# subtotechnoblade/Grok_Alpha_Zero

Measured on AMD Instinct MI355X. Metric: self-play positions/sec (whole node), Connect4 200 sims/move, 1/2/4/8 GPU, higher is better.
Workload: dtype bf16; 1 GPU; Connect4 6x7, 4096 concurrent games/GPU, 200 sims/move (MCTS.run iteration_limit), 6-block x128 ResNet bf16, puct self-play, random-init weights; games_per_gpu=4096, sims_per_move=200, evaluator=resnet

## Files before the change

grok_alpha_zero_amd/build.py:

```python
import os
import subprocess
from concurrent.futures import ThreadPoolExecutor

_PKG = os.path.dirname(os.path.abspath(__file__))
CSRC = os.path.join(_PKG, "csrc")
OBJ = os.path.join(CSRC, "build")
LIB = os.path.join(_PKG, "libgaz_engine.so")
HEADER = os.path.join(os.path.dirname(_PKG), "include", "gaz_engine.h")
UNITS = {
    "engine.hip": ["rt.hpp", "wave.hpp", "det.hpp", "games.hpp", "tree.hpp", "puct_core.hpp", "gumbel_core.hpp", "evaluator.hpp", "samples.hpp", "tree_export.hpp"],
    "resnet.hip": ["rt.hpp", "wave.hpp", "evaluator.hpp", "netops.hpp", "conv3x3.hpp", "conv_wide.hpp", "resblock.hpp", "trunk.hpp", "tile_perm.hpp", "net_host.hpp",
                   "det.hpp", "games.hpp", "tree.hpp", "puct_core.hpp", "gumbel_core.hpp"],
}
FLAGS = ["-O3", "--offload-arch=gfx950", "-fPIC", "-std=c++17", "-ffp-contract=off", "-Wno-unused-result", "-Wno-unused-value",
         "-Wno-int-to-pointer-cast"]


def _newer(target, deps):
    if not os.path.exists(target):
        return True
    t = os.path.getmtime(target)
    return any(os.path.getmtime(d) > t for d in deps)


def build_engine(force=False, verbose=False):
    hipcc = os.environ.get("HIPCC", "/opt/rocm/bin/hipcc")
    os.makedirs(OBJ, exist_ok=True)
    known = {h for hs in UNITS.values() for h in hs} | set(UNITS)
    extra = [f for f in os.listdir(CSRC) if f.endswith((".hpp", ".hip")) and f not in known]
    jobs = []
    for src, hdrs in UNITS.items():
        obj = os.path.join(OBJ, src.replace(".hip", ".o"))
        deps = [os.path.join(CSRC, src), HEADER, os.path.abspath(__file__)] + [os.path.join(CSRC, h) for h in hdrs + extra]
        if force or _newer(obj, deps):
            jobs.append([hipcc] + FLAGS + ["-c", os.path.join(CSRC, src), "-o", obj])

    def run(cmd):
        if verbose:
            print(" ".join(cmd), flush=True)
        subprocess.check_call(cmd, cwd=CSRC)
    with ThreadPoolExecutor(max_workers=max(len(jobs), 1)) as ex:
        list(ex.map(run, jobs))
    objs = [os.path.join(OBJ, s.replace(".hip", ".o")) for s in UNITS]
    if jobs or _newer(LIB, objs):
        run([hipcc, "--offload-arch=gfx950", "-shared", "-fPIC"] + objs + ["-o", LIB])
# ... 2 lines not shown
```

grok_alpha_zero_amd/csrc/engine.hip:

```cpp
#include <stdio.h>
#include <functional>
#include <string>
#include <vector>
#include "../../include/gaz_engine.h"
#include "rt.hpp"
#include "puct_core.hpp"
#include "gumbel_core.hpp"
#include "samples.hpp"
#include "tree_export.hpp"
#include "evaluator.hpp"

using namespace gaz;

static std::string g_create_error;

#define HIP_OK(expr)                                                                  \
    do { hipError_t _e = (expr); if (_e != hipSuccess) { return fail(std::string(#expr) + ": " + hipGetErrorString(_e)); } } while (0)

template <class G> GAZ_DEV void wave_body(const DevParams<G>& E, int g0, int g1) {
    constexpr int PER = WAVE / G::TEAM;
    GAZ_SHARED Scratch<G> S[PER];
    GAZ_SHARED PuctLocal<G> L[PER];
    const int t = team_in_wave<G>();
    const int g = g0 + block_id() * PER + t;
    if (g < g1) game_step<G>(E, g, S[t], L[t]);
}
template <class G> GAZ_KERNEL k_wave(DevParams<G> E, int g0, int g1) { wave_body<G>(E, g0, g1); }
template <class G> GAZ_KERNEL_TEAMS k_wave_teams(DevParams<G> E, int g0, int g1) { wave_body<G>(E, g0, g1); }

template <class G> GAZ_DEV void wave_body_lb(const DevParams<G>& E, const LeafBatch& B, int g0, int g1) {
    constexpr int PER = WAVE / G::TEAM;
    GAZ_SHARED Scratch<G> S[PER];
    GAZ_SHARED PuctLocal<G> L[PER];
    const int t = team_in_wave<G>();
    const int g = g0 + block_id() * PER + t;
    if (g < g1) game_step_lb<G>(E, B, g, S[t], L[t]);
}
template <class G> GAZ_KERNEL_TEAMS k_wave_lb(DevParams<G> E, LeafBatch B, int g0, int g1) { wave_body_lb<G>(E, B, g0, g1); }

template <class G> GAZ_KERNEL k_gather_pending_lb(DevParams<G> E, int K, int32_t* out) {
    const int g = block_id();
    if (g >= E.n_games) return;
    const GameState<G>& gs = E.games[g];
    const int n = gs.pend_kind == PEND_ROOT ? 1 : (gs.pend_kind == PEND_EXPAND ? gs.pend_depth : 0);
    for (int j = lane_id(); j < K; j += WAVE) out[(size_t)g * K + j] = j < n ? gs.pend_kind : PEND_NONE;
}

template <class G> GAZ_KERNEL k_count_reserved(DevParams<G> E, unsigned long long* out) {
    const int g = block_id();
    if (g >= E.n_games) return;
    unsigned long long sum = 0;
    for (int t = 0; t < 2; ++t) {
        const int n = (int)E.trees[(size_t)g * 2 + t].n_nodes;
        for (int i = lane_id(); i < n; i += WAVE) sum += node_at(E, g, t, i).hdr()->pad[0];
    }
    if (sum) atomic_add(out, sum);
}

template <class G> GAZ_DEV void wave_body_gumbel(const DevParams<G>& E, int g0, int g1) {
    constexpr int PER = WAVE / G::TEAM;
    GAZ_SHARED Scratch<G> S[PER];
    GAZ_SHARED GumbelLocal<G> L[PER];
    const int t = team_in_wave<G>();
    const int g = g0 + block_id() * PER + t;
    if (g < g1) g_game_step<G>(E, g, S[t], L[t]);
}
template <class G> GAZ_KERNEL k_wave_gumbel(DevParams<G> E, int g0, int g1) { wave_body_gumbel<G>(E, g0, g1); }
template <class G> GAZ_KERNEL_TEAMS k_wave_gumbel_teams(DevParams<G> E, int g0, int g1) { wave_body_gumbel<G>(E, g0, g1); }

template <class G> GAZ_DEV void wave_body_gb(const DevParams<G>& E, const GumbelBatch& B, int g0, int g1) {
    constexpr int PER = WAVE / G::TEAM;
    GAZ_SHARED Scratch<G> S[PER];
    GAZ_SHARED GumbelLocal<G> L[PER];
    const int t = team_in_wave<G>();
    const int g = g0 + block_id() * PER + t;
    if (g < g1) g_game_step_gb<G>(E, B, g, S[t], L[t]);
}
template <class G> GAZ_KERNEL_TEAMS k_wave_gb(DevParams<G> E, GumbelBatch B, int g0, int g1) { wave_body_gb<G>(E, B, g0, g1); }

template <class G> GAZ_KERNEL k_gather_pending_gb(DevParams<G> E, GumbelBatch B, int32_t* out) {
    const int g = block_id();
    if (g >= E.n_games) return;
    const int kind = E.games[g].pend_kind;
    for (int j = lane_id(); j < B.K; j += WAVE)
        out[(size_t)g * B.K + j] = kind == PEND_ROOT ? (j == 0 ? PEND_ROOT : PEND_NONE) : (kind == PEND_EXPAND && B.rows[(size_t)g * B.K + j].pend ? PEND_EXPAND : PEND_NONE);
}

template <class G> GAZ_KERNEL k_cache_insert(DevParams<G> E, int g0, int g1) {
    const int g = g0 + block_id();
    if (g < g1) cache_insert<G>(E, g);
}

template <int UNUSED> GAZ_KERNEL_WIDE k_init_puct_table(double* table, double c_init, double c_base, int n) {
#ifdef GAZ_HOST_EMU
    for (int i = 0; i < n; ++i) { table[2 * i] = dsqrt((double)i); table[2 * i + 1] = puct_c_of((double)i, c_init, c_base); }
#else
    const int i = blockIdx.x * blockDim.x + threadIdx.x;
    if (i < n) { table[2 * i] = dsqrt((double)i); table[2 * i + 1] = puct_c_of((double)i, c_init, c_base); }
#endif
}

template <class G> GAZ_KERNEL k_init_games(DevParams<G> E, int first_seq) {
    const int g = block_id();
    if (g >= E.n_games || lane_id() != 0) return;
    GameState<G>& gs = E.games[g];
    memset(&gs, 0, sizeof(gs));
    gs.phase = (E.games_budget > 0 && (long long)g >= E.games_budget) ? PH_HALT : PH_NEW_GAME;
    gs.pend_kind = PEND_NONE; gs.game_seq = (uint32_t)first_seq; gs.host_move = -1; gs.winner = RUNNING;
    gs.slot_id = E.slot_offset + (uint32_t)g;
    E.trees[g * 2].root = -1; E.trees[g * 2 + 1].root = -1;
}

template <class G> GAZ_KERNEL k_reset_games(DevParams<G> E, const int32_t* slots, int n) {
    const int i = block_id();
    if (i >= n || lane_id() != 0) return;
    const int g = slots ? slots[i] : i;
    if (g < 0 || g >= E.n_games) return;
    GameState<G>& gs = E.games[g];
// ... 343 lines not shown
        if (dalloc(&E.paths, rows * PathCap<G>::V)) return 1;
        if (lbk > 1 && gbk <= 1) { LB.K = lbk; if (dalloc(&LB.pend, rows)) return 1; }
        if (gbk > 1) { GB.K = gbk; if (dalloc(&GB.rows, rows)) return 1; }
        if (gumbel) { GumbelState<G>* gp = nullptr; if (dalloc(&gp, (size_t)n)) return 1; E.gstate = gp; }
        if (dalloc(&E.recs, (size_t)n * RL::SIZE)) return 1;
        if (dalloc(&E.ring, (size_t)(cfg.ring_capacity > 0 ? cfg.ring_capacity : 1) * RL::SIZE)) return 1;
        if (dalloc(&E.ring_head, 4)) return 1;
        if (dalloc(&E.nn_in, rows * G::HW * G::C + 64)) return 1;
        if (dalloc(&E.nn_policy, rows * G::A + 64)) return 1;
        if (dalloc(&E.nn_value, rows + 64)) return 1;
        if (cfg.eval_cache_log2 < 0 || cfg.eval_cache_log2 > 28) return fail("eval_cache_log2 out of range (0 = off, at most 28)");
        if (cfg.eval_cache_log2 > 0) {
            const size_t slots = (size_t)1 << cfg.eval_cache_log2;
            E.cache_stride = CacheLayout<G>::SIZE; E.cache_mask = (uint32_t)(slots - 1); E.cache_epoch = 1;
            if (dalloc(&E.cache, slots * (size_t)E.cache_stride)) return 1;
            if (dalloc(&E.cache_lock, slots)) return 1;
        }
        if (getenv("GAZ_TREE_PROF") && atoi(getenv("GAZ_TREE_PROF"))) { if (dalloc(&E.prof, (size_t)n * 8)) return 1; }
        if (!gumbel) {
            double* tb = nullptr;
            if (dalloc(&tb, (size_t)2 * PUCT_TABLE_N)) return 1;
            E.puct_table = tb;
            if (init_puct_table()) return 1;
        }
        if (dalloc(&E.stats, 8)) return 1;
        if (dalloc(&E.error, 4)) return 1;
        if (dalloc(&dN, (size_t)n * G::A) || dalloc(&dW, (size_t)n * G::A) || dalloc(&dP, (size_t)n * G::A) ||
            dalloc(&dPol, (size_t)n * G::A) || dalloc(&dRV, n) || dalloc(&dQ, n) || dalloc(&dChosen, n) ||
            dalloc(&dPhase, n) || dalloc(&dPending, rows) || dalloc(&dCount, 16) || dalloc(&dMoves, (size_t)n + G::MAXT) || dalloc(&dSlots, n)) return 1;
        std::string e2;
        gaz_engine_config ecfg = cfg; ecfg.n_games = (int32_t)rows;
        eval = make_evaluator(ecfg, G::H, G::W, G::C, G::A, &e2);
        if (!eval && cfg.evaluator != GAZ_EVAL_EXTERNAL) return fail("evaluator: " + e2);
        GAZ_LAUNCH(k_init_games<G>, n, WAVE, stream, E, (int)cfg.first_game_seq);
        HIP_OK(hipGetLastError());
        HIP_OK(hipStreamSynchronize(stream));
        return 0;
    }

    void note_grouped() override { if (eval) eval->set_shared_chip(this->grouped > 1); }

    int check_device_error() {
        int32_t code = 0;
        HIP_OK(hipMemcpy(&code, E.error, sizeof(code), hipMemcpyDeviceToHost));
        if (code) {
            const char* names[] = {"", "tree arena full (raise nodes_per_tree)", "root not fully expanded at move end",
                                   "selection path longer than the game can last", "state-machine loop guard", "PUCT picked an un-poppable child"};
            return fail(std::string("device error: ") + (code > 0 && code < 6 ? names[code] : "unknown"));
        }
        return 0;
    }

    int load_weights(const gaz_tensor* t, int n) override {
        if (!eval) return fail("no evaluator to load weights into");
        std::string m;
        if (eval->load(t, n, stream, &m)) return fail("load_weights: " + m);
        if (E.cache) {
            HIP_OK(hipMemsetAsync(E.cache, 0, ((size_t)E.cache_mask + 1) * (size_t)E.cache_stride, stream));
            HIP_OK(hipStreamSynchronize(stream));
        }
        return 0;
    }

    int reset_games(const int32_t* slots, int n) override {
        if (slots && n_eff != E.n_games) return fail("reset_games(slots): not after gaz_engine_repack (a physical slot no longer identifies a game; reset all games instead)");
        if (!slots) n_eff = E.n_games;
// ... 113 lines not shown
        int n_active = 0;
        for (int g = 0; g < n_eff; ++g) n_active += ph[g] != PH_HALT;
        for (int g = n_eff; g < E.n_games; ++g) if (ph[g] != PH_HALT) return fail("repack: a slot beyond the live range is running");
        if (n_active_out) *n_active_out = n_active;
        const int n_new = n_active > 0 ? n_active : 1;
        std::vector<int32_t> mv;
        int hole = 0;
        for (int g = n_eff - 1; g >= n_new; --g) {
            if (ph[g] == PH_HALT) continue;
            while (hole < n_new && ph[hole] != PH_HALT) ++hole;
            if (hole >= n_new) return fail("repack: internal error (no hole left)");
            mv.push_back(g); mv.push_back(hole); ph[hole] = ph[g]; ph[g] = PH_HALT;
        }
        if (!mv.empty()) {
            if (!dMoveList && dalloc(&dMoveList, (size_t)2 * E.n_games)) return 1;
            HIP_OK(hipMemcpyAsync(dMoveList, mv.data(), mv.size() * 4, hipMemcpyHostToDevice, stream));
            const size_t slot_bytes = (size_t)2 * (E.compact ? 2 : 1) * (size_t)E.nodes_per_tree * (size_t)E.node_bytes;
            const size_t gbytes = cfg.search == GAZ_SEARCH_GUMBEL ? sizeof(GumbelState<G>) : 0;
#ifdef GAZ_HOST_EMU
            DevParams<G> Em = E; Em.eval_done = d_evaldone;
            GAZ_LAUNCH(k_move_slots<G>, (int)(mv.size() / 2), 1, stream, Em, (const int32_t*)dMoveList, (int)(mv.size() / 2), slot_bytes, gbytes);
#else
            DevParams<G> Em = E; Em.eval_done = d_evaldone;
            GAZ_LAUNCH(k_move_slots<G>, (int)(mv.size() / 2), 256, stream, Em, (const int32_t*)dMoveList, (int)(mv.size() / 2), slot_bytes, gbytes);
#endif
            HIP_OK(hipGetLastError());
            HIP_OK(hipStreamSynchronize(stream));
        }
        n_eff = n_new;
        if (n_eff_out) *n_eff_out = n_eff;
        return 0;
    }

    int one_wave(bool with_eval) {
        ++waves_launched;
        if (with_eval && eval && fuse_enabled && can_fuse()) {
            const bool timing = this->timing && n_waves_total % TIMING_STRIDE == 0 && ev.size() + 4 <= MAX_TIMING_EVENTS;
            static const char* stamp_spec = getenv("GAZ_FUSED_STAMPS");
            static const long stamp_at = stamp_spec && strchr(stamp_spec, ':') ? atol(strchr(stamp_spec, ':') + 1) : 3000;
            unsigned long long* d_stamps = nullptr;
            const size_t stamp_blocks = (size_t)n_eff + 4096;
            if (stamp_spec && n_waves_total == stamp_at && hipMalloc((void**)&d_stamps, stamp_blocks * 128 * 8) == hipSuccess) hipMemsetAsync(d_stamps, 0, stamp_blocks * 128 * 8, stream);
            const FuseHandoff ho{d_done, fuse_epoch + 1, d_evaldone, d_fault, SPIN_TICKS, debug_fault_mod, d_stamps, d_queue};
            const void* plan = eval->trunk_plan(E.nn_in, n_eff, 0, ho);
            if (plan) {
                hipEvent_t e0 = 0, e1 = 0, e2 = 0;
                if (timing) { e0 = new_event(); e1 = new_event(); e2 = new_event(); hipEventRecord(e0, stream); }
                DevParams<G> Ef = wave_params(); Ef.done_flag = d_done;
                if (eval->plan_uses_queue(plan)) {
                    typedef typename PuctVariant<G>::type GPq;
                    static const bool gumbel_teams = !(getenv("GAZ_FUSE_GUMBEL_TEAMS") && atoi(getenv("GAZ_FUSE_GUMBEL_TEAMS")) == 0);
                    static const int rounds_env = getenv("GAZ_FUSE_TREE_ROUNDS") ? atoi(getenv("GAZ_FUSE_TREE_ROUNDS")) : 0;
                    const int rounds = rounds_env > 0 ? rounds_env : (G::ID == GAME_GMK ? (this->grouped > 1 ? 4 : 8) : (cfg.search == GAZ_SEARCH_GUMBEL ? (this->grouped > 1 ? 2 : 4) : 1));
                    const int gpb = G::ID == GAME_GMK ? rounds * 8 : rounds * 4 * ((cfg.search == GAZ_SEARCH_GUMBEL && !gumbel_teams) ? 1 : WAVE / GPq::TEAM);
                    Ef.done_queue = d_queue; Ef.queue_gpb = gpb; Ef.queue_nfull = n_eff / gpb; Ef.queue_rem = n_eff % gpb;
                }
                Ef.handoff_release = G::ID == GAME_GMK;
                const bool launched = G::ID == GAME_GMK ? launch_wave_trunk_gmk(stream, &Ef, 0, n_eff, plan)
                                    : cfg.search == GAZ_SEARCH_GUMBEL ? launch_wave_trunk_c4_gumbel(stream, &Ef, 0, n_eff, plan) : launch_wave_trunk_c4(stream, &Ef, 0, n_eff, plan);
                if (!launched) {
                    fuse_state = 0; --fuse_epoch;
                    return one_wave(with_eval);
                }
                prev_marked = true;
                if (d_stamps) {
                    std::vector<unsigned long long> hst(stamp_blocks * 128);
                    hipStreamSynchronize(stream);
                    hipMemcpy(hst.data(), d_stamps, hst.size() * 8, hipMemcpyDeviceToHost); hipFree(d_stamps);
                    std::string path(stamp_spec); if (path.find(':') != std::string::npos) path = path.substr(0, path.find(':'));
                    if (FILE* f = fopen(path.c_str(), "wb")) { fwrite(hst.data(), 8, hst.size(), f); fclose(f); }
                }
                if (timing) hipEventRecord(e1, stream);
                eval->forward_heads(stream, E.nn_policy, E.nn_value, n_eff, 0);
                if (E.cache) { Ef.eval_done = d_evaldone; GAZ_LAUNCH(k_cache_insert<G>, n_eff, WAVE, stream, Ef, 0, n_eff); E.cache_epoch++; }
                if (timing) {
                    hipEventRecord(e2, stream); ev_eval.push_back({e0, e2}); n_waves_timed++;
                    ev_fused.push_back({e0, e1});
                }
                n_waves_total++;
                return 0;
            }
        }
        const bool timing = this->timing && n_waves_total % TIMING_STRIDE == 0 && ev.size() + 4 <= MAX_TIMING_EVENTS;
        hipEvent_t e0 = 0, e1 = 0, e2 = 0;
        if (timing) { e0 = new_event(); e1 = new_event(); e2 = new_event(); hipEventRecord(e0, stream); }
        DevParams<G> P = wave_params();
        launch_wave(stream, 0, n_eff, P);
        prev_marked = false;
        if (timing) hipEventRecord(e1, stream);
        if (with_eval && eval) eval->forward(stream, E.nn_in, E.nn_policy, E.nn_value, n_eff * lbk, timing);
        if (timing) { hipEventRecord(e2, stream); ev_tree.push_back({e0, e1}); ev_eval.push_back({e1, e2}); n_waves_timed++; }
        P.eval_done = nullptr;
        if (with_eval && eval && debug_fault_mod && d_evaldone) {
            GAZ_LAUNCH(k_debug_skip<G>, n_eff, WAVE, stream, P, d_evaldone, n_eff, debug_fault_mod, d_fault);
            prev_marked = true; P.eval_done = d_evaldone;
        }
        if (with_eval && eval && E.cache) { GAZ_LAUNCH(k_cache_insert<G>, n_eff, WAVE, stream, P, 0, n_eff); E.cache_epoch++; }
        n_waves_total++;
        return 0;
    }

    hipStream_t tstream = 0, hstream = 0;
    static constexpr int MAXGRP = 8;
    int n_grp = 0, grp0[MAXGRP + 1] = {};
    hipEvent_t ev_tree_done[2][MAXGRP] = {}, ev_trunk_done[2][MAXGRP] = {}, ev_heads_done[2][MAXGRP] = {}, ev_join = 0;
    bool pipeline_ready = false;
    bool can_pipeline() {
        static const char* spec = getenv("GAZ_PIPELINE");
        if (!spec || !*spec || atoi(spec) == 0) return false;
        if (lbk > 1 || E.sync_moves || !eval || !eval->supports_split() || E.n_games < 1024 || E.cache || n_eff != E.n_games) return false;
        if (!pipeline_ready) {
            std::vector<int> sizes;
            if (strchr(spec, ',')) { for (const char* p = spec; *p;) { sizes.push_back(atoi(p)); p = strchr(p, ','); if (!p) break; ++p; } }
            else { const int round = eval->round_rows(); for (int left = E.n_games; left > 0; left -= round) sizes.push_back(left < round ? left : round); }
            int sum = 0; for (int v : sizes) sum += v;
            if (sizes.size() < 2 || sizes.size() > (size_t)MAXGRP || sum != E.n_games) return false;
            for (int v : sizes) if (v <= 0) return false;
            n_grp = (int)sizes.size(); grp0[0] = 0;
            for (int i = 0; i < n_grp; ++i) grp0[i + 1] = grp0[i] + sizes[i];
            int lo = 0, hi = 0;
// ... 855 lines not shown
    return 0;
}
int gaz_engine_read_trees(gaz_engine* h, const int32_t* slots, int32_t n_slots, int32_t tree, int32_t max_depth, uint32_t min_visits, int64_t max_nodes,
                          int64_t max_edges, gaz_tree_node* nodes, gaz_tree_edge* edges, int64_t* node_first, int64_t* edge_first) {
    if (n_slots < 0) return h->fail("read_trees: n_slots must be >= 0, not " + std::to_string(n_slots));
    if (!node_first || !edge_first || (n_slots > 0 && !slots)) return h->fail("read_trees: slots, node_first and edge_first must not be null");
    if (check_tree_arg(h, "read_trees", tree)) return 1;
    if ((nodes == nullptr) != (edges == nullptr)) return h->fail("read_trees: nodes and edges must both be given, or both be null (counting call)");
    if (nodes && (max_nodes < 0 || max_edges < 0)) return h->fail("read_trees: max_nodes and max_edges must be >= 0");
    for (int32_t i = 0; i < n_slots; ++i)
        if (slots[i] < 0 || slots[i] >= h->cfg.n_games)
            return h->fail("read_trees: slots[" + std::to_string(i) + "] = " + std::to_string(slots[i]) + " is out of range [0, " + std::to_string(h->cfg.n_games) + ")");
    const gaz_engine::TreePlace place = [&](int64_t nn, int64_t ne, gaz_tree_node** pn, gaz_tree_edge** pe) {
        if (nn > max_nodes || ne > max_edges) return h->short_capacity(nn, ne, max_nodes, max_edges);
        *pn = nodes; *pe = edges; return 0;
    };
    return h->read_trees(slots, n_slots, tree, max_depth, min_visits, node_first, edge_first, nodes != nullptr, place);
}
int gaz_engine_read_pv(gaz_engine* h, int32_t tree, const int32_t* first_action, int32_t max_len, uint8_t* actions, uint32_t* N, float* W, int32_t* len) {
    if (max_len <= 0) return h->fail("read_pv: max_len must be positive, not " + std::to_string(max_len));
    if (!actions || !N || !W || !len) return h->fail("read_pv: actions, N, W and len must not be null");
    if (check_tree_arg(h, "read_pv", tree)) return 1;
    return h->read_pv(tree, first_action, max_len, actions, N, W, len);
}
int gaz_engine_repack(gaz_engine* h, int32_t* n_active, int32_t* n_launch) { return h->repack(n_active, n_launch); }
int gaz_engine_read_head_features(gaz_engine* h, int32_t n, float* p, float* v, int32_t* p_row, int32_t* v_row) { return h->read_head_features(n, p, v, p_row, v_row); }
int gaz_engine_probe_rules(gaz_engine* h, const int32_t* actions, const int32_t* n_actions, int32_t n_positions, int32_t stride, int8_t* board,
                           uint8_t* legal, int32_t* winner, int8_t* input, int32_t* terminal, const float* policy_in, float* policy_out) {
    return h->probe_rules(actions, n_actions, n_positions, stride, board, legal, winner, input, terminal, policy_in, policy_out);
}
int gaz_engine_dominant_kernel(gaz_engine* h, char* name, int32_t cap, double* flops) { return h->dominant(name, cap, flops); }
int gaz_engine_timing_get(gaz_engine* h, double* a, double* b, double* c, int64_t* d, int64_t* e) { return h->timing_get(a, b, c, d, e); }

}
```

grok_alpha_zero_amd/csrc/evaluator.hpp:

```cpp
#pragma once
#include <string>
#include "../../include/gaz_engine.h"
#include "rt.hpp"

namespace gaz {

struct FuseHandoff { const unsigned* ready; unsigned epoch; unsigned* eval_done; int* fuse_fault; unsigned spin_ticks; unsigned test_fault_mod;
                     unsigned long long* stamps;
                     const unsigned long long* queue; };

struct Evaluator {
    virtual ~Evaluator() {}
    virtual int load(const gaz_tensor* t, int n, hipStream_t s, std::string* err) { (void)t; (void)n; (void)s; (void)err; return 0; }
    virtual void forward(hipStream_t s, const int8_t* in, float* policy, float* value, int n, bool timing, int p0 = 0) = 0;
    virtual bool supports_row_base() const { return false; }
    virtual bool supports_split() const { return false; }
    virtual int round_rows() const { return 0; }
    virtual void forward_trunk(hipStream_t s, const int8_t* in, int n, bool timing, int p0) { (void)s; (void)in; (void)n; (void)timing; (void)p0; }
    virtual void forward_heads(hipStream_t s, float* policy, float* value, int n, int p0) { (void)s; (void)policy; (void)value; (void)n; (void)p0; }
    virtual const void* trunk_plan(const int8_t* in, int n, int p0, const struct FuseHandoff& h) { (void)in; (void)n; (void)p0; (void)h; return nullptr; }
    virtual bool plan_uses_queue(const void* plan) const { (void)plan; return false; }
    virtual void set_shared_chip(bool on) { (void)on; }
    virtual bool ready() const { return true; }
    virtual void timing_reset() {}
    virtual void timing_get(double* ms, int64_t* launches) { *ms = 0; *launches = 0; }
    virtual const char* dominant_kernel(int n, double* flops) { (void)n; *flops = 0; return ""; }
    virtual bool head_features(const float** p_feat, const float** v_feat, int* p_row_floats, int* v_row_floats) { (void)p_feat; (void)v_feat; (void)p_row_floats; (void)v_row_floats; return false; }
};

GAZ_DEV uint32_t hash_row(const int8_t* s, int n, uint32_t seed) {
    uint32_t h = 2166136261u ^ seed;
    for (int i = 0; i < n; ++i) { h ^= (uint8_t)s[i]; h *= 16777619u; }
    h ^= h >> 16; h *= 0x85EBCA6Bu; h ^= h >> 13; h *= 0xC2B2AE35u; h ^= h >> 16;
    return h;
}

template <int UNUSED> GAZ_KERNEL_WIDE k_hash_eval(const int8_t* in, float* policy, float* value, int n, int row_bytes, int A, uint32_t salt) {
#ifdef GAZ_HOST_EMU
// ... 45 lines not shown
```

grok_alpha_zero_amd/csrc/net_host.hpp:

```cpp
#pragma once
#include <map>
#include <string>
#include <type_traits>
#include <vector>
#include "evaluator.hpp"
#include "conv3x3.hpp"
#include "conv_wide.hpp"
#include "netops.hpp"
#include "trunk.hpp"

namespace gaz {

inline bool env_on(const char* name, bool dflt) { const char* v = getenv(name); return v ? atoi(v) != 0 : dflt; }
inline int env_int(const char* name, int dflt) { const char* v = getenv(name); return v ? atoi(v) : dflt; }

inline bf16_t f2bf_host(float f) { unsigned u; memcpy(&u, &f, 4); return (bf16_t)((u + 0x7FFFu + ((u >> 16) & 1u)) >> 16); }

enum ConvOrder { CONV_MFMA, CONV_WIDE };
struct DeviceStore {
    std::vector<void*> allocs; std::string err;
    std::map<std::string, const gaz_tensor*> by; std::map<std::string, float*> f32; std::map<std::string, bf16_t*> b16;
    ~DeviceStore() { for (void* p : allocs) hipFree(p); }
    static constexpr size_t PAD = 64;
    template <class T> T* dalloc(size_t n) {
        void* p = nullptr;
        if (hipMalloc(&p, (n + PAD) * sizeof(T)) != hipSuccess) { err = "hipMalloc"; return nullptr; }
        allocs.push_back(p); return (T*)p;
    }
    template <class T> T* upload(const T* h, size_t n) { T* d = dalloc<T>(n); if (d) hipMemcpy(d, h, n * sizeof(T), hipMemcpyHostToDevice); return d; }
    void set_tensors(const gaz_tensor* t, int n) { by.clear(); for (int i = 0; i < n; ++i) by[t[i].name] = &t[i]; }
    const gaz_tensor* need(const std::string& name, int64_t numel) {
        auto it = by.find(name);
        if (it == by.end()) { err = "missing tensor " + name; return nullptr; }
        if (it->second->numel != numel) { err = "tensor " + name + " has " + std::to_string(it->second->numel) + " elements, expected " + std::to_string(numel); return nullptr; }
        return it->second;
    }
    float* g(const std::string& name) const { auto it = f32.find(name); return it == f32.end() ? nullptr : it->second; }
    bf16_t* w(const std::string& name) const { auto it = b16.find(name); return it == b16.end() ? nullptr : it->second; }
    bool up_f32(const std::string& name, int64_t numel) { const gaz_tensor* t = need(name, numel); return t && (f32[name] = upload(t->data, (size_t)numel)) != nullptr; }
    bool up_conv(const std::string& name, int cout, int cin, int ntaps, ConvOrder order) {
        const int64_t numel = (int64_t)ntaps * cout * cin;
        const gaz_tensor* t = need(name, numel); if (!t) return false;
        std::vector<bf16_t> h(numel);
        if (order == CONV_WIDE) arrange_wide_weights(t->data, cout, cin, ntaps, h.data(), f2bf_host);
        else arrange_conv_weights(t->data, cout, cin, h.data(), f2bf_host, ntaps);
        return (b16[name] = upload(h.data(), h.size())) != nullptr;
    }
// ... 102 lines not shown
```

grok_alpha_zero_amd/csrc/puct_core.hpp:

```cpp
#pragma once
#include "det.hpp"
#include "tree.hpp"

namespace gaz {

template <class G> struct PathCap { static constexpr int V = (G::MAXT + 3 + 7) / 8 * 8; };

struct PathEnt { int32_t node; int32_t slot; };

template <class G> struct DevParams {
    int32_t n_games, run_iterations, max_actions, explore_first, explore_second;
    int32_t create_new_root, sync_moves, nodes_per_tree, ring_cap, use_dirichlet, max_tree_sims;
    double c_init, c_base, alpha, eps;
    double c_visit, c_scale;
    int32_t gumbel_m, node_bytes, compact;
    int32_t stop_search;
    uint64_t move_time_ticks;
    int32_t fast_find_win;
    int32_t g_stablemax;
    int32_t single_tree;
    double tau;
    int32_t no_gumbel_noise;
    uint32_t first_game_seq;
    long long games_budget;
    int32_t n_opening, opening_actions[8];
    int32_t fast_iterations;
    double opening_weights[8];
    double full_search_prob;
    double forced_playouts_k;
    float one_minus_eps;
    uint32_t key0, key1, slot_offset;
    uint8_t* arena;
    TreeState* trees;
    GameState<G>* games;
    void* gstate;
    PathEnt* paths;
    uint8_t* recs;
    uint8_t* ring;
    uint32_t* ring_head;
    int8_t* nn_in;
    float* nn_policy;
    float* nn_value;
    uint8_t* cache; uint32_t* cache_lock; uint32_t cache_mask, cache_epoch; int32_t cache_stride;
    unsigned long long* stats;
    const double* puct_table;
    unsigned long long* prof;
    int32_t* error;
    uint32_t* done_flag;
    uint32_t wave_epoch;
    uint32_t* eval_done;
    int32_t handoff_release;
    unsigned long long* done_queue;
    int32_t queue_gpb, queue_nfull, queue_rem;
};

struct PendLeaf { int32_t parent, slot, node, depth; };
struct LeafBatch {
    int32_t K;
    PendLeaf* pend;
};

GAZ_DEV void store_coherent(int* p, int v) {
#ifdef GAZ_HOST_EMU
    *p = v;
#else
    __hip_atomic_store(p, v, __ATOMIC_RELAXED, __HIP_MEMORY_SCOPE_SYSTEM);
#endif
}

#ifdef GAZ_HOST_EMU
#define GAZ_PROF(k, t0) do { } while (0)
#define GAZ_PROF_NOW() 0ll
#else
#define GAZ_PROF_NOW() (E.prof ? (long long)clock64() : 0ll)
#define GAZ_PROF(k, t0) do { if (E.prof && tlane<G>() == 0) E.prof[(size_t)g * 8 + (k)] += (unsigned long long)((long long)clock64() - (t0)); } while (0)
#endif

enum : int32_t { ERR_ARENA_FULL = 1, ERR_ROOT_NOT_EXPANDED = 2, ERR_PATH_OVERFLOW = 3, ERR_LOOP_GUARD = 4, ERR_BAD_SELECT = 5 };

template <class G> struct Scratch {
    int8_t board[G::BPAD];
    uint8_t legal[G::APAD];
    uint8_t tact[G::APAD];
    uint8_t twin[G::APAD];
    uint8_t sact[G::APAD];
    float pri[G::APAD];
// ... 1070 lines not shown
            }
            wave_sync();
            bool ended = winner != RUNNING;
            int todo = 0;
            if (!ended) {
                if (prune<G>(E, g, trees[0], 0, action)) todo |= 1;
                if (!E.single_tree && prune<G>(E, g, trees[1], 1, action)) todo |= 2;
            }
            if (ply + 1 == E.max_actions) { winner = 0; ended = true; }
            if (!ended && tlane<G>() == 0) { gs.roots_todo = todo; gs.phase = (E.sync_moves && E.single_tree) ? PH_IDLE : PH_ROOT; }
            if (ended) {
                if (tlane<G>() == 0) {
                    gs.winner = winner;
                    int32_t* hdr = reinterpret_cast<int32_t*>(rec);
                    hdr[0] = ply + 1; hdr[1] = winner; hdr[2] = (int32_t)gs.slot_id; hdr[3] = (int32_t)gs.game_seq;
                    atomic_max(&E.stats[0], (unsigned long long)(ply + 1));
                    atomic_add(&E.stats[1], (unsigned long long)(ply + 1));
                    atomic_add(&E.stats[2], 1ull);
                    atomic_add(&E.stats[winner + 4], 1ull);
                    gs.phase = PH_RING_WAIT;
                }
            }
            wave_sync();
        } else if (phase == PH_RING_WAIT) {
            if (!ring_push<G>(E, g, gs)) return true;
            if (E.sync_moves) return true;
        } else {
            return true;
        }
        return false;
    };
    bool done = false;
    for (int guard = 0; guard < 100000; ++guard) {
        if (!done && phase_step()) { fin(); done = true; }
        if (!ballot(!done)) return;
    }
    set_error(E.error, ERR_LOOP_GUARD);
    if (!done) fin();
}


template <class G> struct PuctLocal { GameState<G> gs; TreeState ts[2]; };

template <class G, class T> GAZ_DEV void copy_state_words(T* dst, const T* src) {
    static_assert(sizeof(T) % 4 == 0, "word copy");
    uint32_t* d = reinterpret_cast<uint32_t*>(dst); const uint32_t* s = reinterpret_cast<const uint32_t*>(src);
    for (int i = tlane<G>(); i < (int)(sizeof(T) / 4); i += G::TEAM) d[i] = s[i];
}

template <class G> GAZ_DEV void publish_done(const DevParams<G>& E, int g, uint32_t* block_rank = nullptr, int block = 0) {
#ifndef GAZ_HOST_EMU
    if (E.done_queue && block_rank) {
        asm volatile("s_waitcnt vmcnt(0)" ::: "memory");
        if (E.handoff_release) {
            if (tlane<G>() == 0) __builtin_amdgcn_fence(__ATOMIC_RELEASE, "agent");
            asm volatile("s_waitcnt vmcnt(0)" ::: "memory");
        }
        if (tlane<G>() == 0) {
            const int rank = (int)atomic_add(block_rank, 1u);
            const int entry = rank * E.queue_nfull + (rank < E.queue_rem ? rank : E.queue_rem) + block;
            __hip_atomic_store(E.done_queue + entry, ((unsigned long long)E.wave_epoch << 32) | (unsigned)g, __ATOMIC_RELAXED, __HIP_MEMORY_SCOPE_SYSTEM);
        }
        return;
    }
    if (!E.done_flag) return;
    if (E.handoff_release) {
        asm volatile("s_waitcnt vmcnt(0)" ::: "memory");
        if (tlane<G>() == 0) __builtin_amdgcn_fence(__ATOMIC_RELEASE, "agent");
    }
    asm volatile("s_waitcnt vmcnt(0)" ::: "memory");
    if (tlane<G>() == 0) store_coherent(reinterpret_cast<int*>(E.done_flag + g), (int)E.wave_epoch);
#endif
}

template <class G> GAZ_DEV bool eval_was_skipped(const DevParams<G>& E, int g) {
    if (!E.eval_done) return false;
    return tuni<G>(E.eval_done[g]) != E.wave_epoch - 1;
}

template <class G> GAZ_DEV void game_step(const DevParams<G>& E, int g, Scratch<G>& S, PuctLocal<G>& L, uint32_t* block_rank = nullptr, int block = 0) {
    GameState<G>* gsG = &E.games[g];
    TreeState* tsG = E.trees + (size_t)g * 2;
    if (eval_was_skipped<G>(E, g)) { publish_done<G>(E, g, block_rank, block); return; }
    if (E.compact) { game_step_body<G>(E, g, S, *gsG, tsG, [&]() { publish_done<G>(E, g, block_rank, block); }); return; }
    const long long tw0 = GAZ_PROF_NOW();
    copy_state_words<G>(&L.gs, gsG); copy_state_words<G>(&L.ts[0], &tsG[0]); copy_state_words<G>(&L.ts[1], &tsG[1]);
    wave_sync();
    game_step_body<G>(E, g, S, L.gs, L.ts, [&]() {
        wave_sync();
        copy_state_words<G>(gsG, &L.gs); copy_state_words<G>(&tsG[0], &L.ts[0]); copy_state_words<G>(&tsG[1], &L.ts[1]);
        publish_done<G>(E, g, block_rank, block);
        GAZ_PROF(6, tw0);
    });
}

template <class G> GAZ_DEV void game_step_lb(const DevParams<G>& E, const LeafBatch& B, int g, Scratch<G>& S, PuctLocal<G>& L) {
    GameState<G>* gsG = &E.games[g];
    TreeState* tsG = E.trees + (size_t)g * 2;
    if (E.compact) { game_step_body<G, true>(E, g, S, *gsG, tsG, []() {}, B); return; }
    copy_state_words<G>(&L.gs, gsG); copy_state_words<G>(&L.ts[0], &tsG[0]); copy_state_words<G>(&L.ts[1], &tsG[1]);
    wave_sync();
    game_step_body<G, true>(E, g, S, L.gs, L.ts, [&]() {
        wave_sync();
        copy_state_words<G>(gsG, &L.gs); copy_state_words<G>(&tsG[0], &L.ts[0]); copy_state_words<G>(&tsG[1], &L.ts[1]);
    }, B);
}

}
```

grok_alpha_zero_amd/csrc/resnet.hip:

```cpp
#include <math.h>
#include <map>
#include <string>
#include <vector>
#include <algorithm>
#include "evaluator.hpp"
#include "conv3x3.hpp"
#include "conv_wide.hpp"
#include "netops.hpp"
#include "resblock.hpp"
#include "trunk.hpp"
#include "tile_perm.hpp"
#include "net_host.hpp"
#include "puct_core.hpp"
#include "gumbel_core.hpp"

namespace gaz {

struct Rb3Plan { int tm, halo, tile_rows; };
static Rb3Plan rb3_plan(int M, int H, int W, int n_cus) {
    Rb3Plan best{3, W + 1, 64 * 3 - 2 * (W + 1)}; double best_cost = 1e30;
    for (int aligned = 0; aligned < 2; ++aligned)
        for (int c = 2; c <= 4; ++c) {
            const int rows = aligned ? (64 * c / (H * W)) * (H * W) : 64 * c - 2 * (W + 1);
            if (rows <= 0) continue;
// ... 1090 lines not shown
    hipFuncSetAttribute((const void*)(k_trunk_mix<8, 2, true, true>), hipFuncAttributeMaxDynamicSharedMemorySize, (int)trunk_lds_bytes(128));
    hipFuncSetAttribute((const void*)(k_trunk<2, 2, 8, 2, true, true, false, true>), hipFuncAttributeMaxDynamicSharedMemorySize, (int)trunk_lds_bytes(128));
    hipFuncSetAttribute((const void*)(k_trunk_mix<8, 2, true, true, true>), hipFuncAttributeMaxDynamicSharedMemorySize, (int)trunk_lds_bytes(128));
    hipFuncSetAttribute((const void*)(k_trunk_mix<8, 2, true, true, true, true>), hipFuncAttributeMaxDynamicSharedMemorySize, (int)trunk_lds_bytes(128));
    hipFuncSetAttribute((const void*)(k_trunk<2, 2, 8, 2, false, false>), hipFuncAttributeMaxDynamicSharedMemorySize, (int)trunk_lds_bytes(128));
    hipFuncSetAttribute((const void*)(k_conv3x3<128, 128, 256, 4, 2, 2, 2, 1, 1, 0>), hipFuncAttributeMaxDynamicSharedMemorySize, 160 * 1024);
    hipFuncSetAttribute((const void*)(k_conv3x3<128, 128, 128, 2, 2, 2, 2, 2, 2, 0>), hipFuncAttributeMaxDynamicSharedMemorySize, 160 * 1024);
    return e;
}

}

namespace gaz {

typedef TeamGame<GAME_C4> GP4;

#ifndef GAZ_TREE_ROLE_ATTR
#define GAZ_TREE_ROLE_ATTR __forceinline__
#endif
template <class GP, class LOCAL, bool GUMBEL, int THREADS = TR_THREADS, size_t LDS_BYTES = trunk_lds_bytes(96)>
__device__ GAZ_TREE_ROLE_ATTR void tree_role(const DevParams<GP>& E, int g0, int g1, uint4* lds) {
    constexpr int PER = WAVE / GP::TEAM, NT = (THREADS / WAVE) * PER;
    Scratch<GP>* S = reinterpret_cast<Scratch<GP>*>(lds);
    LOCAL* L = reinterpret_cast<LOCAL*>(S + NT);
    uint32_t* rank = reinterpret_cast<uint32_t*>(L + NT);
    static_assert(NT * (sizeof(Scratch<GP>) + sizeof(LOCAL)) + 16 <= LDS_BYTES, "tree scratch must fit the trunk's LDS allocation");
    if (E.done_queue) {
        if (threadIdx.x == 0) *rank = 0;
        __syncthreads();
    }
    const int w = threadIdx.x >> 6, t = team_in_wave<GP>(), i = w * PER + t;
    const int per_block = E.done_queue ? E.queue_gpb : NT;
    for (int r = 0; r * NT < per_block; ++r) {
        const int g = g0 + (int)blockIdx.x * per_block + r * NT + w * PER + t;
        if (g < g1) {
            if constexpr (GUMBEL) g_game_step<GP>(E, g, S[i], L[i], rank, (int)blockIdx.x);
            else game_step<GP>(E, g, S[i], L[i], rank, (int)blockIdx.x);
        }
    }
}

template <bool MIX, bool SKIP, class GP, class LOCAL, bool GUMBEL>
__device__ __forceinline__ void wave_trunk_body(const DevParams<GP>& E, int g0, int g1, int n_tree_blocks, const TrunkArgs& a) {
    if ((int)blockIdx.x < n_tree_blocks) {
        extern __shared__ uint4 lds[];
        const DevParams<GP> El = E;
        if (a.stamps && (threadIdx.x & 63) == 0) a.stamps[(size_t)blockIdx.x * 128 + (threadIdx.x >> 6)] = wall_clock64();
        tree_role<GP, LOCAL, GUMBEL>(El, g0, g1, lds);
        if (a.stamps && (threadIdx.x & 63) == 0) a.stamps[(size_t)blockIdx.x * 128 + 4 + (threadIdx.x >> 6)] = wall_clock64();
        return;
    }
    const int bid = (int)blockIdx.x - n_tree_blocks;
    if (MIX && bid >= a.n_big) trunk_tile<3, 4, 8, true, true, false, true, 4, false, SKIP ? 2 : 0>(a, (long)a.n_big * a.tile_rows + (long)(bid - a.n_big) * a.small_rows, a.small_rows, SKIP ? a.perm_small : nullptr, a.boff_small);
    else trunk_tile<2, 2, 8, true, true, false, true, 4, false, SKIP ? 1 : 0>(a, (long)bid * a.tile_rows, a.tile_rows, SKIP ? a.perm : nullptr, a.boff);
}

template <bool MIX, bool SKIP> __global__ __launch_bounds__(TR_THREADS, 2) void k_wave_trunk(DevParams<GP4> E, int g0, int g1, int n_tree_blocks, TrunkArgs a) {
    wave_trunk_body<MIX, SKIP, GP4, PuctLocal<GP4>, false>(E, g0, g1, n_tree_blocks, a);
}

typedef Game<GAME_GMK> GGMK;
__global__ __launch_bounds__(512, 1) void k_wave_trunk_gmk(DevParams<GGMK> E, int g0, int g1, int n_tree_blocks, TrunkArgs a) {
    if ((int)blockIdx.x < n_tree_blocks) {
        extern __shared__ uint4 lds[];
        if (a.stamps && (threadIdx.x & 63) == 0) a.stamps[(size_t)blockIdx.x * 128 + (threadIdx.x >> 6)] = wall_clock64();
        tree_role<GGMK, PuctLocal<GGMK>, false, 512, trunk_lds_bytes_s0()>(E, g0, g1, lds);
        if (a.stamps && (threadIdx.x & 63) == 0) a.stamps[(size_t)blockIdx.x * 128 + 8 + (threadIdx.x >> 6)] = wall_clock64();
        return;
// ... 43 lines not shown
```

Measured before the change: 67150 positions/s.

## Order game-to-block assignment by per-game simulation-cost estimate to balance tree work

Adds a per-game EMA of simulations per step, recorded when each game finishes a step. A single-block counting-sort kernel bins games by estimated cost and spreads each class across positions. The tree-search kernels then map block slots through this permutation, so expensive games are spread evenly across wavefronts and blocks instead of clustering. This aims to reduce tail imbalance within the fused tree plus trunk wave. The cost is an extra sort kernel per wave, an indirection load per game, and less contiguous memory access.

```diff
diff --git a/grok_alpha_zero_amd/build.py b/grok_alpha_zero_amd/build.py
--- a/grok_alpha_zero_amd/build.py
+++ b/grok_alpha_zero_amd/build.py
@@ -8,9 +8,9 @@
 LIB = os.path.join(_PKG, "libgaz_engine.so")
 HEADER = os.path.join(os.path.dirname(_PKG), "include", "gaz_engine.h")
 UNITS = {
-    "engine.hip": ["rt.hpp", "wave.hpp", "det.hpp", "games.hpp", "tree.hpp", "puct_core.hpp", "gumbel_core.hpp", "evaluator.hpp", "samples.hpp", "tree_export.hpp"],
+    "engine.hip": ["rt.hpp", "wave.hpp", "det.hpp", "games.hpp", "tree.hpp", "puct_core.hpp", "gumbel_core.hpp", "evaluator.hpp", "samples.hpp", "tree_export.hpp", "tree_order.hpp"],
     "resnet.hip": ["rt.hpp", "wave.hpp", "evaluator.hpp", "netops.hpp", "conv3x3.hpp", "conv_wide.hpp", "resblock.hpp", "trunk.hpp", "tile_perm.hpp", "net_host.hpp",
-                   "det.hpp", "games.hpp", "tree.hpp", "puct_core.hpp", "gumbel_core.hpp"],
+                   "det.hpp", "games.hpp", "tree.hpp", "puct_core.hpp", "gumbel_core.hpp", "tree_order.hpp"],
 }
 FLAGS = ["-O3", "--offload-arch=gfx950", "-fPIC", "-std=c++17", "-ffp-contract=off", "-Wno-unused-result", "-Wno-unused-value",
          "-Wno-int-to-pointer-cast"]
diff --git a/grok_alpha_zero_amd/csrc/engine.hip b/grok_alpha_zero_amd/csrc/engine.hip
--- a/grok_alpha_zero_amd/csrc/engine.hip
+++ b/grok_alpha_zero_amd/csrc/engine.hip
@@ -22,8 +22,8 @@
     GAZ_SHARED Scratch<G> S[PER];
     GAZ_SHARED PuctLocal<G> L[PER];
     const int t = team_in_wave<G>();
-    const int g = g0 + block_id() * PER + t;
-    if (g < g1) game_step<G>(E, g, S[t], L[t]);
+    const int i = block_id() * PER + t;
+    if (i < g1 - g0) game_step<G>(E, g0 + (E.order ? E.order[i] : i), S[t], L[t]);
 }
 template <class G> GAZ_KERNEL k_wave(DevParams<G> E, int g0, int g1) { wave_body<G>(E, g0, g1); }
 template <class G> GAZ_KERNEL_TEAMS k_wave_teams(DevParams<G> E, int g0, int g1) { wave_body<G>(E, g0, g1); }
@@ -84,6 +84,27 @@
     const int kind = E.games[g].pend_kind;
     for (int j = lane_id(); j < B.K; j += WAVE)
         out[(size_t)g * B.K + j] = kind == PEND_ROOT ? (j == 0 ? PEND_ROOT : PEND_NONE) : (kind == PEND_EXPAND && B.rows[(size_t)g * B.K + j].pend ? PEND_EXPAND : PEND_NONE);
+}
+
+#ifdef GAZ_HOST_EMU
+constexpr int ORDER_THREADS = 1;
+#else
+constexpr int ORDER_THREADS = 256;
+#endif
+template <int NT> GAZ_KERNEL_WIDE k_order_games(const uint16_t* hint, int n, int32_t* order, int class_shift, int per_wave) {
+    GAZ_SHARED OrderScratch<NT> S;
+#ifdef GAZ_HOST_EMU
+    order_games<NT>(hint, n, order, S, 0, class_shift, per_wave);
+#else
+    order_games<NT>(hint, n, order, S, (int)threadIdx.x, class_shift, per_wave);
+#endif
+}
+template <int UNUSED> GAZ_KERNEL k_junk_hints(uint16_t* hint, int n, uint32_t wave) {
+    const int g = block_id();
+    if (g >= n || lane_id() != 0) return;
+    uint32_t x = (uint32_t)g * 2654435761u ^ (wave + 1u) * 40503u;
+    x ^= x >> 15; x *= 2246822519u; x ^= x >> 13;
+    hint[g] = (wave % 3u == 0u) ? (uint16_t)0xffffu : (uint16_t)x;
 }
 
 template <class G> GAZ_KERNEL k_cache_insert(DevParams<G> E, int g0, int g1) {
@@ -493,6 +514,7 @@
         gaz_engine_config ecfg = cfg; ecfg.n_games = (int32_t)rows;
         eval = make_evaluator(ecfg, G::H, G::W, G::C, G::A, &e2);
         if (!eval && cfg.evaluator != GAZ_EVAL_EXTERNAL) return fail("evaluator: " + e2);
+        if (init_tree_order()) return 1;
         GAZ_LAUNCH(k_init_games<G>, n, WAVE, stream, E, (int)cfg.first_game_seq);
         HIP_OK(hipGetLastError());
         HIP_OK(hipStreamSynchronize(stream));
@@ -672,6 +694,72 @@
         return 0;
     }
 
+    bool order_on = false, order_junk = false, order_apply = true; int order_every = 1, order_seg_shift = 0, order_class_shift = COST_CLASS_SHIFT, order_fixed = 0, order_spread = 1; int64_t order_wave = 0;
+    uint16_t* d_step_cost = nullptr; int32_t* d_order = nullptr; int order_n = 0;
+    uint16_t* d_cost_log = nullptr; long cost_log_first = 0, cost_log_count = 0, cost_log_have = 0; std::string cost_log_path;
+    int init_tree_order() {
+        order_on = G::ID == GAME_C4 && cfg.search == GAZ_SEARCH_PUCT && lbk == 1 && env_on("GAZ_TREE_ORDER", true);
+        if (!order_on) return 0;
+        order_junk = env_on("GAZ_TREE_ORDER_JUNK", false);
+        order_apply = env_on("GAZ_TREE_ORDER_APPLY", true);
+        order_class_shift = env_int("GAZ_TREE_ORDER_CLASS_SHIFT", COST_CLASS_SHIFT); if (order_class_shift < 0 || order_class_shift > 15) order_class_shift = COST_CLASS_SHIFT;
+        order_fixed = env_int("GAZ_TREE_ORDER_FIXED", 0);
+        order_spread = env_int("GAZ_TREE_ORDER_SPREAD", 4); if (order_spread < 1 || order_spread > 64) order_spread = 1;
+        order_every = env_int("GAZ_TREE_ORDER_EVERY", 1); if (order_every < 1) order_every = 1;
+        order_seg_shift = env_int("GAZ_TREE_ORDER_SEG_SHIFT", 0); if (order_seg_shift < 0 || order_seg_shift > 30) order_seg_shift = 0;
+        if (dalloc(&d_step_cost, (size_t)E.n_games) || dalloc(&d_order, (size_t)E.n_games)) return 1;
+        if (const char* spec = getenv("GAZ_TREE_ORDER_DUMP")) {
+            cost_log_path = spec; cost_log_first = 3000; cost_log_count = 300;
+            const size_t c1 = cost_log_path.find(':');
+            if (c1 != std::string::npos) {
+                const std::string rest = cost_log_path.substr(c1 + 1); cost_log_path = cost_log_path.substr(0, c1);
+                cost_log_first = atol(rest.c_str());
+                if (rest.find(':') != std::string::npos) cost_log_count = atol(rest.c_str() + rest.find(':') + 1);
+            }
+            if (cost_log_count < 1 || cost_log_count > 4096) cost_log_count = 300;
+            cost_log_path += "." + std::to_string(cfg.slot_offset);
+            if (dalloc(&d_cost_log, (size_t)cost_log_count * E.n_games)) return 1;
+        }
+        return 0;
+    }
+    void take_order() {
+        if (order_junk) GAZ_LAUNCH(k_junk_hints<0>, n_eff, WAVE, stream, d_step_cost, n_eff, (uint32_t)waves_launched);
+        if (order_fixed) {
+            if (order_n != n_eff) {
+                std::vector<int32_t> h(n_eff);
+                for (int i = 0; i < n_eff; ++i) h[i] = i;
+                uint32_t x = 12345u;
+                if (order_fixed == 2) for (int i = n_eff - 1; i > 0; --i) { x = x * 1664525u + 1013904223u; const int j = (int)((x >> 8) % (uint32_t)(i + 1)); std::swap(h[i], h[j]); }
+                hipMemcpy(d_order, h.data(), (size_t)n_eff * 4, hipMemcpyHostToDevice);
+                order_n = n_eff;
+            }
+            return;
+        }
+        GAZ_LAUNCH(k_order_games<ORDER_THREADS>, 1, ORDER_THREADS, stream, (const uint16_t*)d_step_cost, n_eff, d_order, order_class_shift, order_spread);
+        order_n = n_eff;
+    }
+    template <class P> void set_order(P& p) {
+        if (!order_on) return;
+        if (order_n != n_eff) take_order();
+        p.step_cost = d_step_cost; p.order = order_apply ? d_order : nullptr;
+    }
+    void order_next() {
+        if (!order_on) return;
+        if (d_cost_log && n_waves_total >= cost_log_first && cost_log_have < cost_log_count) {
+            hipMemcpyAsync(d_cost_log + (size_t)cost_log_have * E.n_games, d_step_cost, (size_t)E.n_games * 2, hipMemcpyDeviceToDevice, stream);
+            if (++cost_log_have == cost_log_count) {
+                std::vector<uint16_t> h((size_t)cost_log_count * E.n_games);
+                hipStreamSynchronize(stream);
+                hipMemcpy(h.data(), d_cost_log, h.size() * 2, hipMemcpyDeviceToHost);
+                if (FILE* f = fopen(cost_log_path.c_str(), "wb")) {
+                    const int32_t hdr[4] = {0x54524f43, (int32_t)cost_log_count, E.n_games, n_eff};
+                    fwrite(hdr, 4, 4, f); fwrite(h.data(), 2, h.size(), f); fclose(f);
+                }
+            }
+        }
+        if (++order_wave % order_every == 0) take_order();
+    }
+
     int one_wave(bool with_eval) {
         ++waves_launched;
         if (with_eval && eval && fuse_enabled && can_fuse()) {
@@ -687,6 +775,7 @@
                 hipEvent_t e0 = 0, e1 = 0, e2 = 0;
                 if (timing) { e0 = new_event(); e1 = new_event(); e2 = new_event(); hipEventRecord(e0, stream); }
                 DevParams<G> Ef = wave_params(); Ef.done_flag = d_done;
+                set_order(Ef);
                 if (eval->plan_uses_queue(plan)) {
                     typedef typename PuctVariant<G>::type GPq;
                     static const bool gumbel_teams = !(getenv("GAZ_FUSE_GUMBEL_TEAMS") && atoi(getenv("GAZ_FUSE_GUMBEL_TEAMS")) == 0);
@@ -694,6 +783,7 @@
                     const int rounds = rounds_env > 0 ? rounds_env : (G::ID == GAME_GMK ? (this->grouped > 1 ? 4 : 8) : (cfg.search == GAZ_SEARCH_GUMBEL ? (this->grouped > 1 ? 2 : 4) : 1));
                     const int gpb = G::ID == GAME_GMK ? rounds * 8 : rounds * 4 * ((cfg.search == GAZ_SEARCH_GUMBEL && !gumbel_teams) ? 1 : WAVE / GPq::TEAM);
                     Ef.done_queue = d_queue; Ef.queue_gpb = gpb; Ef.queue_nfull = n_eff / gpb; Ef.queue_rem = n_eff % gpb;
+                    Ef.queue_seg_shift = Ef.order ? order_seg_shift : 0;
                 }
                 Ef.handoff_release = G::ID == GAME_GMK;
                 const bool launched = G::ID == GAME_GMK ? launch_wave_trunk_gmk(stream, &Ef, 0, n_eff, plan)
@@ -711,6 +801,7 @@
                     if (FILE* f = fopen(path.c_str(), "wb")) { fwrite(hst.data(), 8, hst.size(), f); fclose(f); }
                 }
                 if (timing) hipEventRecord(e1, stream);
+                order_next();
                 eval->forward_heads(stream, E.nn_policy, E.nn_value, n_eff, 0);
                 if (E.cache) { Ef.eval_done = d_evaldone; GAZ_LAUNCH(k_cache_insert<G>, n_eff, WAVE, stream, Ef, 0, n_eff); E.cache_epoch++; }
                 if (timing) {
@@ -725,7 +816,9 @@
         hipEvent_t e0 = 0, e1 = 0, e2 = 0;
         if (timing) { e0 = new_event(); e1 = new_event(); e2 = new_event(); hipEventRecord(e0, stream); }
         DevParams<G> P = wave_params();
+        set_order(P);
         launch_wave(stream, 0, n_eff, P);
+        order_next();
         prev_marked = false;
         if (timing) hipEventRecord(e1, stream);
         if (with_eval && eval) eval->forward(stream, E.nn_in, E.nn_policy, E.nn_value, n_eff * lbk, timing);
@@ -1647,4 +1740,15 @@
 int gaz_engine_dominant_kernel(gaz_engine* h, char* name, int32_t cap, double* flops) { return h->dominant(name, cap, flops); }
 int gaz_engine_timing_get(gaz_engine* h, double* a, double* b, double* c, int64_t* d, int64_t* e) { return h->timing_get(a, b, c, d, e); }
 
-}
+#ifdef GAZ_HOST_EMU
+int gaz_test_order_games(const uint16_t* hint, int n, int32_t* order, int32_t* cls) {
+    static gaz::OrderScratch<ORDER_THREADS> S;
+    gaz::order_games<ORDER_THREADS>(hint, n, order, S, 0);
+    for (int i = 0; i < n && cls; ++i) cls[i] = gaz::order_class(hint[i]);
+    return gaz::ORDER_CLASSES;
+}
+int gaz_test_spread_position(int p, int n, int per) { return gaz::spread_position(p, n, per); }
+int gaz_test_step_cost_update(int hint, int sims) { return (int)gaz::step_cost_update((uint16_t)hint, sims); }
+#endif
+
+}
diff --git a/grok_alpha_zero_amd/csrc/evaluator.hpp b/grok_alpha_zero_amd/csrc/evaluator.hpp
--- a/grok_alpha_zero_amd/csrc/evaluator.hpp
+++ b/grok_alpha_zero_amd/csrc/evaluator.hpp
@@ -4,6 +4,9 @@
 #include "rt.hpp"
 
 namespace gaz {
+
+inline bool env_on(const char* name, bool dflt) { const char* v = getenv(name); return v ? atoi(v) != 0 : dflt; }
+inline int env_int(const char* name, int dflt) { const char* v = getenv(name); return v ? atoi(v) : dflt; }
 
 struct FuseHandoff { const unsigned* ready; unsigned epoch; unsigned* eval_done; int* fuse_fault; unsigned spin_ticks; unsigned test_fault_mod;
                      unsigned long long* stamps;
diff --git a/grok_alpha_zero_amd/csrc/net_host.hpp b/grok_alpha_zero_amd/csrc/net_host.hpp
--- a/grok_alpha_zero_amd/csrc/net_host.hpp
+++ b/grok_alpha_zero_amd/csrc/net_host.hpp
@@ -11,8 +11,6 @@
 
 namespace gaz {
 
-inline bool env_on(const char* name, bool dflt) { const char* v = getenv(name); return v ? atoi(v) != 0 : dflt; }
-inline int env_int(const char* name, int dflt) { const char* v = getenv(name); return v ? atoi(v) : dflt; }
 
 inline bf16_t f2bf_host(float f) { unsigned u; memcpy(&u, &f, 4); return (bf16_t)((u + 0x7FFFu + ((u >> 16) & 1u)) >> 16); }
 
diff --git a/grok_alpha_zero_amd/csrc/puct_core.hpp b/grok_alpha_zero_amd/csrc/puct_core.hpp
--- a/grok_alpha_zero_amd/csrc/puct_core.hpp
+++ b/grok_alpha_zero_amd/csrc/puct_core.hpp
@@ -1,6 +1,7 @@
 #pragma once
 #include "det.hpp"
 #include "tree.hpp"
+#include "tree_order.hpp"
 
 namespace gaz {
 
@@ -52,6 +53,9 @@
     int32_t handoff_release;
     unsigned long long* done_queue;
     int32_t queue_gpb, queue_nfull, queue_rem;
+    int32_t queue_seg_shift;
+    uint16_t* step_cost;
+    const int32_t* order;
 };
 
 struct PendLeaf { int32_t parent, slot, node, depth; };
@@ -1188,11 +1192,11 @@
     };
     bool done = false;
     for (int guard = 0; guard < 100000; ++guard) {
-        if (!done && phase_step()) { fin(); done = true; }
+        if (!done && phase_step()) { fin(tree_only); done = true; }
         if (!ballot(!done)) return;
     }
     set_error(E.error, ERR_LOOP_GUARD);
-    if (!done) fin();
+    if (!done) fin(tree_only);
 }
 
 
@@ -1214,7 +1218,14 @@
         }
         if (tlane<G>() == 0) {
             const int rank = (int)atomic_add(block_rank, 1u);
-            const int entry = rank * E.queue_nfull + (rank < E.queue_rem ? rank : E.queue_rem) + block;
+            int entry = rank * E.queue_nfull + (rank < E.queue_rem ? rank : E.queue_rem) + block;
+            if (E.queue_seg_shift) {
+                const int first = (block >> E.queue_seg_shift) << E.queue_seg_shift, n_blocks = E.queue_nfull + (E.queue_rem ? 1 : 0);
+                const int cnt = n_blocks - first < (1 << E.queue_seg_shift) ? n_blocks - first : (1 << E.queue_seg_shift);
+                const bool has_partial = E.queue_rem && first + cnt == n_blocks;
+                const int nfull = has_partial ? cnt - 1 : cnt, rem = has_partial ? E.queue_rem : 0;
+                entry = first * E.queue_gpb + rank * nfull + (rank < rem ? rank : rem) + (block - first);
+            }
             __hip_atomic_store(E.done_queue + entry, ((unsigned long long)E.wave_epoch << 32) | (unsigned)g, __ATOMIC_RELAXED, __HIP_MEMORY_SCOPE_SYSTEM);
         }
         return;
@@ -1229,6 +1240,10 @@
 #endif
 }
 
+template <class G> GAZ_DEV void note_step_cost(const DevParams<G>& E, int g, int sims) {
+    if (E.step_cost && tlane<G>() == 0) E.step_cost[g] = step_cost_update(E.step_cost[g], sims);
+}
+
 template <class G> GAZ_DEV bool eval_was_skipped(const DevParams<G>& E, int g) {
     if (!E.eval_done) return false;
     return tuni<G>(E.eval_done[g]) != E.wave_epoch - 1;
@@ -1238,14 +1253,15 @@
     GameState<G>* gsG = &E.games[g];
     TreeState* tsG = E.trees + (size_t)g * 2;
     if (eval_was_skipped<G>(E, g)) { publish_done<G>(E, g, block_rank, block); return; }
-    if (E.compact) { game_step_body<G>(E, g, S, *gsG, tsG, [&]() { publish_done<G>(E, g, block_rank, block); }); return; }
+    if (E.compact) { game_step_body<G>(E, g, S, *gsG, tsG, [&](int sims) { publish_done<G>(E, g, block_rank, block); note_step_cost<G>(E, g, sims); }); return; }
     const long long tw0 = GAZ_PROF_NOW();
     copy_state_words<G>(&L.gs, gsG); copy_state_words<G>(&L.ts[0], &tsG[0]); copy_state_words<G>(&L.ts[1], &tsG[1]);
     wave_sync();
-    game_step_body<G>(E, g, S, L.gs, L.ts, [&]() {
+    game_step_body<G>(E, g, S, L.gs, L.ts, [&](int sims) {
         wave_sync();
         copy_state_words<G>(gsG, &L.gs); copy_state_words<G>(&tsG[0], &L.ts[0]); copy_state_words<G>(&tsG[1], &L.ts[1]);
         publish_done<G>(E, g, block_rank, block);
+        note_step_cost<G>(E, g, sims);
         GAZ_PROF(6, tw0);
     });
 }
@@ -1253,10 +1269,10 @@
 template <class G> GAZ_DEV void game_step_lb(const DevParams<G>& E, const LeafBatch& B, int g, Scratch<G>& S, PuctLocal<G>& L) {
     GameState<G>* gsG = &E.games[g];
     TreeState* tsG = E.trees + (size_t)g * 2;
-    if (E.compact) { game_step_body<G, true>(E, g, S, *gsG, tsG, []() {}, B); return; }
+    if (E.compact) { game_step_body<G, true>(E, g, S, *gsG, tsG, [](int) {}, B); return; }
     copy_state_words<G>(&L.gs, gsG); copy_state_words<G>(&L.ts[0], &tsG[0]); copy_state_words<G>(&L.ts[1], &tsG[1]);
     wave_sync();
-    game_step_body<G, true>(E, g, S, L.gs, L.ts, [&]() {
+    game_step_body<G, true>(E, g, S, L.gs, L.ts, [&](int) {
         wave_sync();
         copy_state_words<G>(gsG, &L.gs); copy_state_words<G>(&tsG[0], &L.ts[0]); copy_state_words<G>(&tsG[1], &L.ts[1]);
     }, B);
diff --git a/grok_alpha_zero_amd/csrc/resnet.hip b/grok_alpha_zero_amd/csrc/resnet.hip
--- a/grok_alpha_zero_amd/csrc/resnet.hip
+++ b/grok_alpha_zero_amd/csrc/resnet.hip
@@ -1146,8 +1146,9 @@
     const int w = threadIdx.x >> 6, t = team_in_wave<GP>(), i = w * PER + t;
     const int per_block = E.done_queue ? E.queue_gpb : NT;
     for (int r = 0; r * NT < per_block; ++r) {
-        const int g = g0 + (int)blockIdx.x * per_block + r * NT + w * PER + t;
-        if (g < g1) {
+        const int idx = (int)blockIdx.x * per_block + r * NT + w * PER + t;
+        if (idx < g1 - g0) {
+            const int g = g0 + (E.order ? E.order[idx] : idx);
             if constexpr (GUMBEL) g_game_step<GP>(E, g, S[i], L[i], rank, (int)blockIdx.x);
             else game_step<GP>(E, g, S[i], L[i], rank, (int)blockIdx.x);
         }
diff --git a/grok_alpha_zero_amd/csrc/tree_order.hpp b/grok_alpha_zero_amd/csrc/tree_order.hpp
--- /dev/null
+++ b/grok_alpha_zero_amd/csrc/tree_order.hpp
@@ -0,0 +1,70 @@
+#pragma once
+#include "wave.hpp"
+
+namespace gaz {
+
+constexpr int ORDER_CLASSES = 16;
+constexpr int COST_FRAC_BITS = 8;
+constexpr int COST_EMA_SHIFT = 2;
+constexpr int COST_CLASS_SHIFT = 6;
+constexpr int COST_MAX_SIMS = 200;
+
+GAZ_HD uint16_t step_cost_update(uint16_t hint, int sims) {
+    const int s = sims < 0 ? 0 : (sims > COST_MAX_SIMS ? COST_MAX_SIMS : sims);
+    const int h = (int)hint, d = (s << COST_FRAC_BITS) - h;
+    const int step = d >= 0 ? (d >> COST_EMA_SHIFT) : -((-d + (1 << COST_EMA_SHIFT) - 1) >> COST_EMA_SHIFT);
+    const int n = h + step;
+    return (uint16_t)(n < 0 ? 0 : (n > 0xffff ? 0xffff : n));
+}
+
+GAZ_HD int order_class(uint16_t hint, int shift = COST_CLASS_SHIFT) {
+    const int over = (int)hint - (1 << COST_FRAC_BITS);
+    const int c = over <= 0 ? 0 : (over >> shift);
+    return c >= ORDER_CLASSES ? ORDER_CLASSES - 1 : c;
+}
+
+GAZ_HD int spread_position(int p, int n, int per) {
+    for (int t = 0; t < per; ++t) {
+        const int cnt = (n - t + per - 1) / per;
+        if (p < cnt) return p * per + t;
+        p -= cnt;
+    }
+    return p;
+}
+
+#ifdef GAZ_HOST_EMU
+inline void block_sync() {}
+#else
+GAZ_DEV void block_sync() { __syncthreads(); }
+#endif
+
+template <int NT> struct OrderScratch {
+    uint32_t cnt[ORDER_CLASSES * NT];
+    uint32_t part[NT];
+};
+
+template <int NT> GAZ_DEV void order_games(const uint16_t* hint, int n, int32_t* order, OrderScratch<NT>& S, int tid, int shift = COST_CLASS_SHIFT, int per = 1) {
+    const int chunk = (n + NT - 1) / NT, s0 = tid * chunk, s1 = s0 + chunk < n ? s0 + chunk : n;
+    for (int c = 0; c < ORDER_CLASSES; ++c) S.cnt[c * NT + tid] = 0;
+    for (int s = s0; s < s1; ++s) S.cnt[order_class(hint[s], shift) * NT + tid] += 1;
+    block_sync();
+    uint32_t sum = 0;
+    for (int i = 0; i < ORDER_CLASSES; ++i) sum += S.cnt[tid * ORDER_CLASSES + i];
+    S.part[tid] = sum;
+    block_sync();
+    for (int d = 1; d < NT; d <<= 1) {
+        const uint32_t add = tid >= d ? S.part[tid - d] : 0u;
+        block_sync();
+        S.part[tid] += add;
+        block_sync();
+    }
+    uint32_t run = S.part[tid] - sum;
+    for (int i = 0; i < ORDER_CLASSES; ++i) { const uint32_t c = S.cnt[tid * ORDER_CLASSES + i]; S.cnt[tid * ORDER_CLASSES + i] = run; run += c; }
+    block_sync();
+    for (int s = s0; s < s1; ++s) {
+        const uint32_t pos = S.cnt[order_class(hint[s], shift) * NT + tid]++;
+        if (pos < (uint32_t)n) order[spread_position((int)pos, n, per)] = s;
+    }
+}
+
+}
```

Measured after the change: 65300 positions/s. 2.8% lower.
